# timoklein/alphazero-gym

Measured on NVIDIA B200. Metric: MCTS simulations/sec (batched trees), higher is better.
Workload: dtype f64 tree statistics + env dynamics / f32 network with exact int8-sliced tensor-core products

## Files before the change

### alphazero_gym_b200/csrc/engine.cu

```cuda
#include <cuda_runtime.h>

#include <cmath>
#include <cstdio>
#include <cstdlib>
#include <cstring>
#include <initializer_list>
#include <map>
#include <string>
#include <tuple>
#include <utility>
#include <vector>

#include "../../include/azg.h"
#include "common.cuh"
#include "env.cuh"
#include "mlp.cuh"
#include "qmlp.cuh"
#include "qmlp2.cuh"
#include "search_wg.cuh"
#include "selfplay.cuh"
#include "tree_continuous.cuh"
#include "tree_discrete.cuh"

static thread_local std::string g_err;
// ... 371 lines not shown
                volatile float tq = w[(size_t)j * H + k] * sc;
                const float tv = tq;
                int32_t q = tv != tv ? 0 : (tv >= 2147483648.0f ? INT32_MAX : (tv <= -2147483648.0f ? INT32_MIN : (int32_t)nearbyintf(tv)));
                const uint32_t t = ((uint32_t)q + 0x8080u) ^ 0x8080u;
                if (natural_rows) {
                    const size_t o = (size_t)(k / 16) * WG_B_KCHUNK + (size_t)(j / 16) * WG_B_STEP + (size_t)(j % 16) * 16 + (k % 16);
                    pl[o] = (int8_t)((t >> 16) & 0xFF);
                    pl[o + 256] = (int8_t)((t >> 8) & 0xFF);
                    pl[o + 512] = (int8_t)(t & 0xFF);
                    continue;
                }
                const size_t o = (size_t)(k / 16) * 2048 + (size_t)qmlp_perm_row(j) * 16 + (k % 16);
                pl[o] = (int8_t)((t >> 16) & 0xFF);
                pl[QMLP_PLANE + o] = (int8_t)((t >> 8) & 0xFF);
                pl[2 * QMLP_PLANE + o] = (int8_t)(t & 0xFF);
            }
        }
        d += 2 * H;
        w += (size_t)H * H + H;
    }
    const float* wv = w;
    const float* bv = w + H;
    const float* wd = w + H + 1;
    const float* bd = wd + (size_t)P * H;
    for (int k = 0; k < H; ++k) {
        d[(size_t)k * PO] = wv[k];
        for (int q = 0; q < P; ++q) d[(size_t)k * PO + 1 + q] = wd[(size_t)q * H + k];
    }
    d += (size_t)H * PO;
    d[0] = bv[0];
    for (int q = 0; q < P; ++q) d[1 + q] = bd[q];
}

extern "C" int azg_set_weights(azg_engine* e, const float* flat, int64_t n, void* stream) {
    if (!e || !flat) return fail(AZG_EINVAL, "null argument");
    if (n != e->n_weights) return fail(AZG_EINVAL, "weight count " + std::to_string(n) + " != expected " + std::to_string(e->n_weights));
    CK(cudaSetDevice(e->cfg.device));
    cudaStream_t st = (cudaStream_t)stream;
    std::vector<float> host(n);
    cudaPointerAttributes at;
    bool on_device = cudaPointerGetAttributes(&at, flat) == cudaSuccess && (at.type == cudaMemoryTypeDevice || at.type == cudaMemoryTypeManaged);
    cudaGetLastError();
    if (on_device) {
        CK(cudaMemcpyAsync(host.data(), flat, n * sizeof(float), cudaMemcpyDeviceToHost, st));
        CK(cudaStreamSynchronize(st));
    } else {
        memcpy(host.data(), flat, n * sizeof(float));
    }
    std::vector<float> packed;
    pack_weights(e, host.data(), packed);
    CK(cudaMemcpyAsync(e->wpack, packed.data(), packed.size() * sizeof(float), cudaMemcpyHostToDevice, st));
    std::vector<int8_t> qd;
    std::vector<float> qf;
    if (e->q8) {
        pack_weights_q8(e, host.data(), qd, qf);
        CK(cudaMemcpyAsync(e->qdigits, qd.data(), qd.size(), cudaMemcpyHostToDevice, st));
        std::vector<int8_t> qn;
        std::vector<float> qf2;
        pack_weights_q8(e, host.data(), qn, qf2, true);
        CK(cudaMemcpyAsync(e->qdigits_nat, qn.data(), qn.size(), cudaMemcpyHostToDevice, st));
        CK(cudaStreamSynchronize(st));
        CK(cudaMemcpyAsync(e->qfl, qf.data(), qf.size() * sizeof(float), cudaMemcpyHostToDevice, st));
    }
    CK(cudaStreamSynchronize(st));
    e->weights_set = true;
    return AZG_OK;
}

extern "C" int azg_set_tapes(azg_engine* e, const float* d_V, const float* d_prior, const float* d_action) {
    if (!e) return fail(AZG_EINVAL, "null engine");
    if (d_V) {
        if (e->cfg.variant == AZG_DISCRETE && !d_prior) return fail(AZG_EINVAL, "discrete tapes need priors");
        if (e->cfg.variant == AZG_CONTINUOUS && !d_action) return fail(AZG_EINVAL, "continuous tapes need actions");
    }
    e->tapeV = d_V;
    e->tapeP = d_V ? d_prior : nullptr;
    e->tapeA = d_V ? d_action : nullptr;
    return AZG_OK;
}

static TreeParams make_params(const azg_engine* e, int B, int64_t tree_id0) {
    TreeParams p;
    memset(&p, 0, sizeof p);
    const azg_config& c = e->cfg;
    p.B = B; p.R = e->R; p.A = c.num_actions; p.K = c.num_components; p.HS = e->HS;
    p.puct_f32 = c.puct_f32; p.v_target = c.v_target; p.use_tape = e->tapeV != nullptr;
    p.c_uct = c.c_uct; p.gamma = c.gamma; p.epsilon = c.epsilon;
    p.reward_step = e->reward_step; p.reward_terminal = e->reward_terminal;
    p.gamma_f32 = (float)c.gamma; p.action_bound = c.action_bound;
    p.seedp = e->d_seed; p.tree_id0 = tree_id0;
    p.drows = e->drows; p.dstate = e->dstate;
    p.crows = e->crows; p.et = e->et; p.ctl = e->ctl; p.BS = e->cfg.max_trees; p.chead = e->chead;
    p.pw_table = e->pw_table;
    p.rcp_tab = e->dtab; p.sqrt_tab = e->dtab + AZG_TAB + 1;
    p.n_rows = e->n_rows; p.draws = e->draws; p.leaf = e->leaf; p.path = e->path; p.dpath = e->dpath; p.ddepth = e->ddepth; p.mt = e->mt; p.tmt = e->tmt; p.rng_mt = e->mt != nullptr;
    p.ctr = e->ctr; p.X = e->X; p.root_state = e->root_state; p.root_n_init = e->root_n_init; p.err = e->err;
    p.tapeV = e->tapeV; p.tapeP = e->tapeP; p.tapeA = e->tapeA;
    p.prof = e->stats + 8;
    return p;
}

static MlpParams make_mlp_params(const azg_engine* e, int n) {
    MlpParams m;
    memset(&m, 0, sizeof m);
    const azg_config& c = e->cfg;
    m.wpack = e->wpack; m.wcount = e->wcount; m.L = c.n_hidden; m.P = e->P; m.PO_PAD = e->PO_PAD;
    m.n = n; m.X = reinterpret_cast<const float*>(e->X); m.xstride = 4; m.mode = 0;
    m.variant = c.variant; m.A = c.num_actions; m.K = c.num_components; m.R = e->R; m.HS = e->HS;
    m.ls_min = c.log_std_min; m.ls_max = c.log_std_max;
    m.leaf = e->leaf; m.drows = e->drows; m.crows = e->crows; m.chead = e->chead; m.evals = e->ctr + (size_t)3 * n;
    m.ctl = e->ctl; m.et = e->et; m.BS = c.max_trees; m.gamma_f32 = (float)c.gamma;
    m.head_dim = azg_head_dim(e);
    m.qdigits = e->qdigits; m.qdigits_nat = e->qdigits_nat; m.qfl = e->qfl; m.qfl_count = e->qfl_count;
    m.stats = e->stats;
    return m;
}

template <typename... KArgs, typename... Args>
static cudaError_t launch_ex(const azg_engine* e, void (*kernel)(KArgs...), int grid, int block, size_t smem, cudaStream_t st, Args&&... args) {
    cudaLaunchConfig_t cfg;
    memset(&cfg, 0, sizeof cfg);
    cfg.gridDim = dim3(grid);
    cfg.blockDim = dim3(block);
    cfg.dynamicSmemBytes = smem;
    cfg.stream = st;
    cfg.attrs = const_cast<cudaLaunchAttribute*>(&e->l2attr);
    cfg.numAttrs = e->l2_on ? 1 : 0;
    return cudaLaunchKernelEx(&cfg, kernel, std::forward<Args>(args)...);
}

template <int H, int S, int ACT>
static cudaError_t launch_mlp_t(const azg_engine* e, const MlpParams& m, cudaStream_t st, bool set_attr) {
    if (set_attr) return cudaFuncSetAttribute(k_mlp<H, S, ACT>, cudaFuncAttributeMaxDynamicSharedMemorySize, (int)e->mlp_smem);
    const int units = (m.n + MLP_UNIT - 1) / MLP_UNIT;
    const int grid = std::max(1, std::min((units + MLP_NGRP - 1) / MLP_NGRP, e->sm_count));
    return launch_ex(e, k_mlp<H, S, ACT>, grid, MLP_THREADS(H), e->mlp_smem, st, m);
}

template <int S, int ACT, int NL>
static cudaError_t launch_qmlp_t(const azg_engine* e, const MlpParams& m, cudaStream_t st, bool set_attr) {
    if (set_attr) {
        cudaError_t ce = cudaFuncSetAttribute(k_qmlp2<S, ACT, NL, false>, cudaFuncAttributeMaxDynamicSharedMemorySize, (int)e->qmlp_smem);
        if (ce != cudaSuccess) return ce;
        ce = cudaFuncSetAttribute(k_qmlp2<S, ACT, NL, true>, cudaFuncAttributeMaxDynamicSharedMemorySize, (int)e->qmlp_smem);
        if (ce != cudaSuccess) return ce;
        if constexpr (S == 4) {
            cudaFuncAttributes fa;
            ce = cudaFuncGetAttributes(&fa, k_qmlp2<S, ACT, NL, true, true>);
            if (ce != cudaSuccess) return ce;
            const_cast<azg_engine*>(e)->tsm_smem_max = e->smem_optin - std::min(e->smem_optin, fa.sharedSizeBytes);
            ce = cudaFuncSetAttribute(k_qmlp2<S, ACT, NL, true, true>, cudaFuncAttributeMaxDynamicSharedMemorySize, (int)e->tsm_smem_max);
            if (ce != cudaSuccess) return ce;
        }
        cudaFuncAttributes fa;
        ce = cudaFuncGetAttributes(&fa, k_search_wg<S, ACT, NL>);
        if (ce != cudaSuccess) return ce;
        if (fa.numRegs * WG_THREADS < WG_EPI_THREADS * WG_EPI_REGS + 128 * WG_MMA_REGS) return cudaErrorLaunchOutOfResources;
        return cudaFuncSetAttribute(k_search_wg<S, ACT, NL>, cudaFuncAttributeMaxDynamicSharedMemorySize, (int)e->wg_smem);
    }
    const int grid = std::max(1, std::min((m.n + 127) / 128, e->sm_count));
    TreeParams none;
    memset(&none, 0, sizeof none);
    return launch_ex(e, k_qmlp2<S, ACT, NL, false>, grid, Q2_THREADS, e->qmlp_smem, st, m, none, 0, 0, 0);
}

template <int S, int ACT, int NL>
static cudaError_t launch_fused_t(const azg_engine* e, const MlpParams& m, const TreeParams& p, int N, cudaStream_t st, int* launches) {
    int chunk = e->sm_count * Q2_MAX_TILES * 128;
    if constexpr (S == 4) {
        int cap = 0;
        while (cap < 128 && qmlp2_tsm_smem_bytes(NL, e->qfl_count, cap + 1, p.R, e->PO_PAD) <= e->tsm_smem_max) ++cap;
        const long long wave = (long long)cap * e->sm_count;
        if (cap > 0 && !p.rng_mt && !getenv("AZG_NO_TSM") && e->fused_mode != 2 && p.B > wave && p.B <= 2 * wave) chunk = (p.B + 1) / 2;
    }
    for (int lo = 0; lo < p.B; lo += chunk) {
        const int hi = std::min(p.B, lo + chunk);
        cudaError_t ce;
        const bool two_phase = e->fused_mode == 1 || (e->fused_mode == 0 && (hi - lo) < 3 * 128 * e->sm_count);
        int tsm_per = 0;
        if constexpr (S == 4) {
            const int per = (hi - lo + e->sm_count - 1) / e->sm_count;
            if (two_phase && !p.rng_mt && !getenv("AZG_NO_TSM") && per <= 128 &&
                qmlp2_tsm_smem_bytes(NL, e->qfl_count, per, p.R, e->PO_PAD) <= e->tsm_smem_max)
                tsm_per = per;
        }
        const_cast<azg_engine*>(e)->last_fused_kind = tsm_per ? 3 : (two_phase ? 1 : 2);
        if (tsm_per) {
            if constexpr (S == 4) {
                const int grid = (hi - lo + tsm_per - 1) / tsm_per;
                ce = launch_ex(e, k_qmlp2<S, ACT, NL, true, true>, grid, Q2_THREADS, qmlp2_tsm_smem_bytes(NL, e->qfl_count, tsm_per, p.R, e->PO_PAD), st, m, p, N, lo, hi);
            }
        } else if (two_phase) {
            const int grid = std::max(1, std::min((hi - lo + 127) / 128, e->sm_count));
            ce = launch_ex(e, k_qmlp2<S, ACT, NL, true>, grid, Q2_THREADS, e->qmlp_smem, st, m, p, N, lo, hi);
        } else {
            const int grid = std::max(1, std::min((hi - lo + 3) / 4, e->sm_count));
            ce = launch_ex(e, k_search_wg<S, ACT, NL>, grid, WG_THREADS, e->wg_smem, st, m, p, N, lo, hi);
        }
        ++*launches;
        if (ce != cudaSuccess) return ce;
    }
    return cudaSuccess;
}

static cudaError_t launch_fused(const azg_engine* e, const MlpParams& m, const TreeParams& p, int N, cudaStream_t st, int* launches) {
    const int S = e->cfg.state_dim, A = e->cfg.activation, NL = e->cfg.n_hidden - 1;
#define FUSED_CASE(s, a, nl) \
    if (S == s && A == a && NL == nl) return launch_fused_t<s, a, nl>(e, m, p, N, st, launches);
    FUSED_CASE(3, 0, 1) FUSED_CASE(3, 1, 1) FUSED_CASE(3, 0, 2) FUSED_CASE(3, 1, 2)
    FUSED_CASE(4, 0, 1) FUSED_CASE(4, 1, 1) FUSED_CASE(4, 0, 2) FUSED_CASE(4, 1, 2)
#undef FUSED_CASE
    return cudaErrorInvalidValue;
}

static cudaError_t launch_mlp(const azg_engine* e, const MlpParams& m, cudaStream_t st, bool set_attr) {
    const int H = e->cfg.hidden, S = e->cfg.state_dim, A = e->cfg.activation;
    if (e->q8) {
        const int NL = e->cfg.n_hidden - 1;
#define QMLP_CASE(s, a, nl) \
    if (S == s && A == a && NL == nl) return launch_qmlp_t<s, a, nl>(e, m, st, set_attr);
        QMLP_CASE(4, 0, 1) QMLP_CASE(4, 1, 1) QMLP_CASE(3, 0, 1) QMLP_CASE(3, 1, 1)
        QMLP_CASE(4, 0, 2) QMLP_CASE(4, 1, 2) QMLP_CASE(3, 0, 2) QMLP_CASE(3, 1, 2)
#undef QMLP_CASE
        return cudaErrorInvalidValue;
    }
#define MLP_CASE(h, s, a) \
    if (H == h && S == s && A == a) return launch_mlp_t<h, s, a>(e, m, st, set_attr);
    MLP_CASE(128, 4, 0) MLP_CASE(128, 4, 1) MLP_CASE(128, 3, 0) MLP_CASE(128, 3, 1)
    MLP_CASE(64, 4, 0) MLP_CASE(64, 4, 1) MLP_CASE(64, 3, 0) MLP_CASE(64, 3, 1)
    MLP_CASE(128, 4, 2) MLP_CASE(128, 4, 3) MLP_CASE(128, 4, 4) MLP_CASE(128, 4, 5)
    MLP_CASE(128, 3, 2) MLP_CASE(128, 3, 3) MLP_CASE(128, 3, 4) MLP_CASE(128, 3, 5)
    MLP_CASE(64, 4, 2) MLP_CASE(64, 4, 3) MLP_CASE(64, 4, 4) MLP_CASE(64, 4, 5)
    MLP_CASE(64, 3, 2) MLP_CASE(64, 3, 3) MLP_CASE(64, 3, 4) MLP_CASE(64, 3, 5)
#undef MLP_CASE
    return cudaErrorInvalidValue;
}

template <bool BK, bool SEL>
static cudaError_t launch_step_continuous(const azg_engine* e, const TreeParams& p, cudaStream_t st) {
    return launch_ex(e, k_step_continuous<BK, SEL>, (p.B + 127) / 128, 128, 0, st, p);
}

struct Prof {
    std::vector<cudaEvent_t> ev;
    std::vector<int> cls;
};

static int enqueue_search(azg_engine* e, int B, int N, int64_t tree_id0, cudaStream_t st, cudaError_t* cerr, Prof* prof = nullptr, bool tree_word = false) {
    TreeParams p = make_params(e, B, tree_word ? 0 : tree_id0);
    p.tree_word = tree_word ? 1 : 0;
    const MlpParams m = make_mlp_params(e, B);
    const bool tape = p.use_tape != 0;
    int launches = 0;
    cudaError_t ce = cudaSuccess;
    auto begin = [&](int cls) {
        if (!prof) return;
        cudaEvent_t a, b;
        cudaEventCreate(&a);
        cudaEventCreate(&b);
        prof->ev.push_back(a);
        prof->ev.push_back(b);
        prof->cls.push_back(cls);
        cudaEventRecord(a, st);
    };
    auto end = [&]() {
        if (prof) cudaEventRecord(prof->ev.back(), st);
    };
#define LK(cls, expr)                                   \
    do {                                                \
        begin(cls);                                     \
        expr;                                           \
        end();                                          \
        ++launches;                                     \
        if (ce == cudaSuccess) ce = cudaGetLastError(); \
    } while (0)
    const int tb = 128, tg = (B + tb - 1) / tb;
    if (e->fused && !tape && !prof) {
        ce = launch_fused(e, m, p, N, st, &launches);
        *cerr = ce;
        return launches;
    }
    if (e->cfg.variant == AZG_DISCRETE) {
        LK(2, (k_init_discrete<<<tg, tb, 0, st>>>(p)));
        if (!tape) LK(1, ce = launch_mlp(e, m, st, false));
        for (int it = 0; it < N; ++it) {
            if (it == 0) LK(0, (k_step_discrete<false, true><<<tg, tb, 0, st>>>(p)));
            else LK(0, (k_step_discrete<true, true><<<tg, tb, 0, st>>>(p)));
            if (!tape) LK(1, ce = launch_mlp(e, m, st, false));
        }
        LK(0, (k_step_discrete<true, false><<<tg, tb, 0, st>>>(p)));
    } else {
        LK(2, (k_init_continuous<<<tg, tb, 0, st>>>(p)));
        if (!tape) LK(1, ce = launch_mlp(e, m, st, false));
        LK(2, (k_root_insert_continuous<<<tg, tb, 0, st>>>(p)));
        for (int it = 0; it < N; ++it) {
            if (it == 0) LK(0, ce = (launch_step_continuous<false, true>(e, p, st)));
            else LK(0, ce = (launch_step_continuous<true, true>(e, p, st)));
            if (!tape) LK(1, ce = launch_mlp(e, m, st, false));
        }
        LK(0, ce = (launch_step_continuous<true, false>(e, p, st)));
    }
#undef LK
    *cerr = ce;
    return launches;
}

static int run_search(azg_engine* e, int B, const double* d_root_state, const int32_t* d_root_n_init, int N, int64_t tree_id0,
                      cudaStream_t st) {
    if (!e) return fail(AZG_EINVAL, "null engine");
    if (B < 1 || B > e->cfg.max_trees) return fail(AZG_EINVAL, "B out of range (max_trees = " + std::to_string(e->cfg.max_trees) + ")");
// ... 539 lines not shown
```

### alphazero_gym_b200/csrc/search_wg.cuh

```cuda
#pragma once
#include "qmlp2.cuh"

#define WG_THREADS 640
#define WG_EPI_THREADS 512
#define WG_IDESC(N) ((2u << 4) | (1u << 7) | (1u << 10) | (((uint32_t)(N) >> 3) << 17) | ((128u >> 4) << 24))
#define WG_B_KCHUNK 6144
#define WG_B_STEP 768
#define WG_WIN_COLS 48
#define WG_STASH_COL 96
#define WG_SLOT_COLS 224
#define WG_MAX_ROUNDS 4

__host__ __device__ inline size_t search_wg_smem_bytes(int NL, int qfl_count) {
    return (size_t)NL * 3 * QMLP_PLANE + 2 * 3 * QMLP_PLANE + (size_t)qfl_count * 4 + 1024 + Q2_TAB_BYTES;
}

__device__ __forceinline__ void umma_i8_wg(uint32_t tmem_d, uint32_t da_lo, uint32_t db_lo, uint32_t idesc, uint32_t accumulate) {
    asm volatile(
        "{\n\t.reg .pred p;\n\t.reg .b64 da, db;\n\tmov.b64 da, {%1, %5};\n\tmov.b64 db, {%2, %5};\n\tsetp.ne.b32 p, %4, 0;\n\t"
        "tcgen05.mma.cta_group::1.kind::i8 [%0], da, db, %3, p;\n\t}" ::"r"(tmem_d),
        "r"(da_lo), "r"(db_lo), "r"(idesc), "r"(accumulate), "r"(Q2_DESC_HI)
        : "memory");
}
__device__ __forceinline__ uint32_t wg_descb_lo(uint32_t saddr) { return ((saddr >> 4) & 0x3FFFu) | (((uint32_t)WG_B_KCHUNK >> 4) << 16); }

#ifndef WG_EPI_REGS
#define WG_EPI_REGS 104
#define WG_MMA_REGS 56
#endif

__device__ __forceinline__ void mbar_arrive_s(uint32_t bar) { asm volatile("mbarrier.arrive.shared::cta.b64 _, [%0];" ::"r"(bar) : "memory"); }
__device__ __forceinline__ bool mbar_try_wait_s(uint32_t bar, uint32_t parity, uint32_t ns) {
    uint32_t ok;
    asm volatile("{\n\t.reg .pred p;\n\tmbarrier.try_wait.parity.shared::cta.b64 p, [%1], %2, %3;\n\tselp.u32 %0, 1, 0, p;\n\t}"
                 : "=r"(ok) : "r"(bar), "r"(parity), "r"(ns) : "memory");
    return ok != 0;
}
__device__ __forceinline__ void mbar_wait_s(uint32_t bar, uint32_t parity) {
    int spins = 0;
    while (!mbar_try_wait_s(bar, parity, 20000u)) {
        if (++spins > (1 << 22)) {
            printf("mbar_wait timeout: block %d thread %d barrier smem 0x%x parity %u\n", blockIdx.x, threadIdx.x, bar, parity);
            __trap();
        }
    }
}

struct WgSlot {
    uint32_t tacc;
    int8_t* sA;
    uint32_t ready, full, accfree, slotfree;
    uint32_t fullph;
    long long cyc_full;
#ifdef AZG_EVAL_PROF
    long long cyc_k[3];
#endif
};

__device__ __forceinline__ float wg_quantise_row(const WgSlot& sl, bool wact, int r, float pm) {
    float cx = 0.0f;
    if (wact) {
        const int e = q8_exponent(pm);
        const float sx = __uint_as_float((uint32_t)(276 - e) << 23);
        cx = __uint_as_float((uint32_t)(e - 22) << 23);
#pragma unroll 2
        for (int c = 0; c < 8; ++c) {
            float v[16];
            tmem_ld16f(sl.tacc + WG_STASH_COL + 16 * c, v);
            tmem_wait_ld();
            q8_store16(v, sx, sl.sA, c, r);
        }
        asm volatile("fence.proxy.async.shared::cta;" ::: "memory");
    }
    tc_fence_before();
    mbar_arrive_s(sl.ready);
    return cx;
}

template <int S, int ACT, int NL>
__device__ __forceinline__ void wg_evaluate(const MlpParams& p, WgSlot& sl, const float* fl, bool wact, bool valid, int gr, int r, float* out) {
    const float* W0 = fl;
    const float* b0 = fl + S * 128;
    const float2* cwb = reinterpret_cast<const float2*>(fl + S * 128 + 128);
    const float* Wh = fl + S * 128 + 128 + NL * 2 * 128;
    const float* bh = Wh + 128 * p.PO_PAD;
    float pm = 0.0f;
    if (wact) {
        float x[S];
#pragma unroll
        for (int s = 0; s < S; ++s) x[s] = 0.0f;
        if (valid) {
            const float4 v = *reinterpret_cast<const float4*>(p.X + (size_t)gr * 4);
            x[0] = v.x; x[1] = v.y; x[2] = v.z;
            if (S > 3) x[S - 1] = v.w;
        }
#pragma unroll 1
        for (int c = 0; c < 8; ++c) {
            float a[16];
#pragma unroll
            for (int i = 0; i < 16; i += 2) {
                const int j = c * 16 + i;
                float2 acc = *reinterpret_cast<const float2*>(b0 + j);
#pragma unroll
                for (int s = 0; s < S; ++s) acc = __ffma2_rn(make_float2(x[s], x[s]), *reinterpret_cast<const float2*>(W0 + s * 128 + j), acc);
                const float2 e = mlp_act2<ACT>(acc);
                a[i] = e.x; a[i + 1] = e.y;
                pm = fmaxf(pm, fmaxf(fabsf(e.x), fabsf(e.y)));
            }
            tmem_st16f(sl.tacc + WG_STASH_COL + 16 * c, a);
        }
        tmem_wait_st();
    }
    float cx = wg_quantise_row(sl, wact, r, pm);
#pragma unroll 1
    for (int l = 0; l < NL; ++l) {
        pm = 0.0f;
#pragma unroll 1
        for (int k = 0; k < 8; ++k) {
            const int w = k & 1;
            const long long f0 = clock64();
            mbar_wait_s(sl.full + 8u * w, (sl.fullph >> w) & 1u);
            sl.fullph ^= 1u << w;
            tc_fence_after();
            sl.cyc_full += clock64() - f0;
#ifdef AZG_EVAL_PROF
            sl.cyc_k[k < 2 ? k : 2] += clock64() - f0;
#endif
            if (wact) {
                const uint32_t ta = sl.tacc + w * WG_WIN_COLS;
                int32_t pa[16], pb[16], pc[16];
                tmem_ld16(ta, pa);
                tmem_ld16(ta + 16, pb);
                tmem_ld16(ta + 32, pc);
                tmem_wait_ld();
                tc_fence_before();
                if (k < 6) mbar_arrive_s(sl.accfree + 8u * w);
                const float2* cb = cwb + l * 128 + 16 * k;
                float v[16];
#pragma unroll
                for (int i = 0; i < 16; i += 2) {
                    const float4 sb = *reinterpret_cast<const float4*>(cb + i);
                    float u0 = __int2float_rn(pa[i] * 256 + pb[i]);
                    float u1 = __int2float_rn(pa[i + 1] * 256 + pb[i + 1]);
                    u0 = __fmaf_rn(u0, 256.0f, q8_i2f_23(pc[i]));
                    u1 = __fmaf_rn(u1, 256.0f, q8_i2f_23(pc[i + 1]));
                    const float2 y = make_float2(__fmaf_rn(u0, __fmul_rn(cx, sb.x), sb.y), __fmaf_rn(u1, __fmul_rn(cx, sb.z), sb.w));
                    const float2 ev = mlp_act2<ACT>(y);
                    v[i] = ev.x; v[i + 1] = ev.y;
                    pm = fmaxf(pm, fmaxf(fabsf(ev.x), fabsf(ev.y)));
                }
                tmem_st16f(sl.tacc + WG_STASH_COL + 16 * k, v);
            } else {
                tc_fence_before();
                if (k < 6) mbar_arrive_s(sl.accfree + 8u * w);
            }
        }
        if (wact) tmem_wait_st();
        if (l + 1 < NL) cx = wg_quantise_row(sl, wact, r, pm);
    }
    if (wact) {
#pragma unroll 1
        for (int c4 = 0; c4 < p.PO_PAD / 4; ++c4) {
            float2 lo[4], hi[4];
#pragma unroll
            for (int q = 0; q < 4; ++q) {
                lo[q] = make_float2(0.0f, 0.0f);
                hi[q] = make_float2(0.0f, 0.0f);
#pragma unroll
                for (int hc = 0; hc < 2; ++hc) {
                    float a[16];
                    tmem_ld16f(sl.tacc + WG_STASH_COL + 32 * q + 16 * hc, a);
                    tmem_wait_ld();
                    const float* wp = Wh + (32 * q + 16 * hc) * p.PO_PAD + c4 * 4;
#pragma unroll
                    for (int i = 0; i < 16; ++i) {
                        const float4 w4 = *reinterpret_cast<const float4*>(wp + i * p.PO_PAD);
                        const float2 av = make_float2(a[i], a[i]);
                        lo[q] = __ffma2_rn(av, make_float2(w4.x, w4.y), lo[q]);
                        hi[q] = __ffma2_rn(av, make_float2(w4.z, w4.w), hi[q]);
                    }
                }
            }
            const float s0 = __fadd_rn(__fadd_rn(__fadd_rn(lo[0].x, lo[1].x), __fadd_rn(lo[2].x, lo[3].x)), bh[c4 * 4 + 0]);
            const float s1 = __fadd_rn(__fadd_rn(__fadd_rn(lo[0].y, lo[1].y), __fadd_rn(lo[2].y, lo[3].y)), bh[c4 * 4 + 1]);
            const float s2 = __fadd_rn(__fadd_rn(__fadd_rn(hi[0].x, hi[1].x), __fadd_rn(hi[2].x, hi[3].x)), bh[c4 * 4 + 2]);
            const float s3 = __fadd_rn(__fadd_rn(__fadd_rn(hi[0].y, hi[1].y), __fadd_rn(hi[2].y, hi[3].y)), bh[c4 * 4 + 3]);
#pragma unroll
            for (int g4 = 0; g4 < Q2_MAX_PO / 4; ++g4)
                if (g4 == c4) { out[4 * g4] = s0; out[4 * g4 + 1] = s1; out[4 * g4 + 2] = s2; out[4 * g4 + 3] = s3; }
        }
    }
    tc_fence_before();
}

template <int S, int ACT, int NL>
__global__ void __launch_bounds__(WG_THREADS, 1)
k_search_wg(const MlpParams p, const TreeParams tp, const int n_sims, const int chunk_begin, const int chunk_end) {
    extern __shared__ __align__(1024) uint8_t wsm_raw[];
    __shared__ __align__(8) uint64_t wbar, ready[2], full[2][2], accfree[2][2], slotfree[2][2];
    __shared__ uint32_t tmem_base_s;
    uint8_t* qsm = wsm_raw + ((1024u - (smem_u32(wsm_raw) & 1023u)) & 1023u);
    int8_t* sB = reinterpret_cast<int8_t*>(qsm);
    int8_t* sA = sB + (size_t)NL * 3 * QMLP_PLANE;
    float* fl = reinterpret_cast<float*>(sA + 2 * 3 * QMLP_PLANE);
    double* s_rcp = reinterpret_cast<double*>(fl + p.qfl_count);
    double* s_sq = s_rcp + FUSED_TAB + 1;
    int32_t* s_pw = reinterpret_cast<int32_t*>(s_sq + FUSED_TAB + 1);

    const int tid = threadIdx.x, warp = tid >> 5, lane = tid & 31;
    const int per = (chunk_end - chunk_begin + gridDim.x - 1) / gridDim.x;
    const int row_begin = chunk_begin + blockIdx.x * per;
    const int row_end = min(row_begin + per, chunk_end);
    if (row_begin >= row_end) return;
    const int nrows = row_end - row_begin;
    const int rounds = (nrows + 511) / 512;
    const int ntiles_max = 4 * rounds;
    int th = (nrows + ntiles_max - 1) / ntiles_max;
    if (th > 32) th = (th + 31) & ~31;
    const int ntiles = (nrows + th - 1) / th;
    const int n_evals = n_sims + 1;

    if (tid == 0) {
        mbar_init(&wbar, 1);
        for (int s = 0; s < 2; ++s) {
            mbar_init(&ready[s], 128);
            mbar_init(&slotfree[s][0], 128);
            mbar_init(&slotfree[s][1], 128);
            for (int w = 0; w < 2; ++w) {
                mbar_init(&full[s][w], 1);
                mbar_init(&accfree[s][w], 128);
            }
        }
    }
    if (warp == 0) {
        asm volatile("tcgen05.alloc.cta_group::1.sync.aligned.shared::cta.b32 [%0], %1;" ::"r"(smem_u32(&tmem_base_s)), "n"(512) : "memory");
        asm volatile("tcgen05.relinquish_alloc_permit.cta_group::1.sync.aligned;" ::: "memory");
    }
    tc_fence_before();
    __syncthreads();
    tc_fence_after();
    const uint32_t tb = tmem_base_s;
#ifdef AZG_WG_DEBUG
    if (tid == 0 && blockIdx.x == 0)
        printf("wg: wbar 0x%x ready 0x%x full 0x%x accfree 0x%x slotfree 0x%x tmem 0x%x nrows %d th %d ntiles %d rounds %d\n", smem_u32(&wbar), smem_u32(ready),
               smem_u32(&full[0][0]), smem_u32(&accfree[0][0]), smem_u32(&slotfree[0][0]), tb, nrows, th, ntiles, rounds);
#endif
    if (tid == 0) {
        const uint32_t bytesB = (uint32_t)NL * 3 * QMLP_PLANE, bytesF = (uint32_t)p.qfl_count * 4u;
        mbar_expect_tx(&wbar, bytesB + bytesF);
        for (uint32_t o = 0; o < bytesB; o += 32768u) bulk_g2s(sB + o, p.qdigits_nat + o, min(32768u, bytesB - o), &wbar);
        bulk_g2s(fl, p.qfl, bytesF, &wbar);
    }
    for (int i = tid; i <= FUSED_TAB; i += blockDim.x) {
        s_rcp[i] = tp.rcp_tab[i];
        s_sq[i] = tp.sqrt_tab[i];
        s_pw[i] = (tp.pw_table && i < p.R) ? tp.pw_table[i] : 0;
    }
    __syncthreads();
    mbar_wait(&wbar, 0);

    if (warp >= 16) {
        asm volatile("setmaxnreg.dec.sync.aligned.u32 %0;" ::"n"(WG_MMA_REGS));
        if (warp < 18) {
            const int slot = warp - 16;
            uint32_t rph = 0, aph = 0;
            const uint32_t aH = q2_desc_lo(smem_u32(sA) + (uint32_t)slot * 3 * QMLP_PLANE), aM = aH + 1024, aL = aH + 2048;
#pragma unroll 1
            for (int s = 0; s < n_evals; ++s)
#pragma unroll 1
            for (int rd = 0; rd < rounds; ++rd)
#pragma unroll 1
            for (int half = 0; half < 2; ++half) {
                if (4 * rd + slot + 2 * half >= ntiles) continue;
#pragma unroll 1
                for (int l = 0; l < NL; ++l) {
#pragma unroll 1
                    for (int k = 0; k < 8; ++k) {
                        const int w = k & 1;
                        if (k == 0) { mbar_wait(&ready[slot], rph); rph ^= 1u; }
                        else if (k >= 2) { mbar_wait(&accfree[slot][w], (aph >> w) & 1u); aph ^= 1u << w; }
                        tc_fence_after();
                        const uint32_t bq = wg_descb_lo(smem_u32(sB) + (uint32_t)l * 3 * QMLP_PLANE + (uint32_t)k * WG_B_STEP);
                        const uint32_t acc = tb + slot * WG_SLOT_COLS + w * WG_WIN_COLS;
                        if (elect_one()) {
#pragma unroll
                        for (int kk = 0; kk < 4; ++kk) {
                            umma_i8_wg(acc, aH + kk * 256, bq + kk * 768, WG_IDESC(48), kk > 0);
                            umma_i8_wg(acc + 16, aM + kk * 256, bq + kk * 768, WG_IDESC(32), 1);
                            umma_i8_wg(acc + 32, aL + kk * 256, bq + kk * 768, WG_IDESC(16), 1);
                        }
                        umma_commit(&full[slot][w]);
                        }
                        __syncwarp();
                    }
                }
            }
        }
    } else {
        asm volatile("setmaxnreg.inc.sync.aligned.u32 %0;" ::"n"(WG_EPI_REGS));
        const int g = warp >> 2, slot = g & 1, half = g >> 1;
        const int r = (warp & 3) * 32 + lane;
        WgSlot sl;
        sl.tacc = tb + ((uint32_t)((warp & 3) * 32) << 16) + slot * WG_SLOT_COLS;
        sl.sA = sA + (size_t)slot * 3 * QMLP_PLANE;
        sl.ready = smem_u32(&ready[slot]); sl.full = smem_u32(full[slot]); sl.accfree = smem_u32(accfree[slot]); sl.slotfree = smem_u32(slotfree[slot]);
        sl.fullph = 0;
        sl.cyc_full = 0;
#ifdef AZG_EVAL_PROF
        sl.cyc_k[0] = sl.cyc_k[1] = sl.cyc_k[2] = 0;
#endif
        bool first_use = true;
        uint32_t useph = 0;
        const Tabs tabs = {s_pw, s_rcp, s_sq, FUSED_TAB};
        long long cyc_tree = 0, cyc_slot = 0;
        const long long cyc_begin = clock64();
        uint32_t nev = 0;
        int ev_row = 0;
        for (int rd = 0; rd < rounds; ++rd) {
            const int tile = 4 * rd + g, row0 = row_begin + tile * th;
            if (tile < ntiles && row0 + r < min(row0 + th, row_end)) {
                if (S == 4) d_init(tp, row0 + r);
                else c_init(tp, row0 + r);
            }
        }
#pragma unroll 1
        for (int s = 0; s < n_evals; ++s) {
#pragma unroll 1
        for (int rd = 0; rd < rounds; ++rd) {
            const int tile = 4 * rd + g;
            const bool tvalid = tile < ntiles;
            const int row0 = row_begin + tile * th;
            const int nv = tvalid ? max(0, min(th, row_end - row0)) : 0;
            const int gr = row0 + r;
            const bool valid = r < nv, wact = (warp & 3) * 32 < nv;
            const long long c0 = clock64();
            if (half == 1 || !first_use) {
                mbar_wait_s(sl.slotfree + 8u * (half ^ 1), useph);
                useph ^= 1u;
            }
            first_use = false;
            tc_fence_after();
            const long long c1 = clock64();
            float out[Q2_MAX_PO];
#pragma unroll
            for (int i = 0; i < Q2_MAX_PO; ++i) out[i] = 0.0f;
            if (tvalid) wg_evaluate<S, ACT, NL>(p, sl, fl, wact, valid, gr, r, out);
            mbar_arrive_s(sl.slotfree + 8u * half);
            const long long c2 = clock64();
            if (valid) {
                int leafw;
                double lr = 0.0;
                if (p.variant == 1) {
                    const uint4 k0 = p.ctl[gr], k1 = p.ctl[(size_t)p.BS + gr];
                    leafw = (int)k0.z;
                    lr = __hiloint2double((int)k1.w, (int)k1.z);
                } else {
                    leafw = p.leaf[gr];
                }
                if (leafw & LEAF_EVAL) {
                    mlp_finish_row(p, gr, leafw, lr, out[0], out + 1);
                    ++nev;
                    ev_row = gr;
                }
                if (S == 4) {
                    d_step(tp, tabs, gr, s > 0, s + 1 < n_evals);
                } else {
                    if (s == 0) c_root_insert(tp, gr);
                    c_step(tp, tabs, gr, s > 0, s + 1 < n_evals);
                }
            }
            cyc_slot += c1 - c0;
            cyc_tree += clock64() - c2;
        }
        }
        if (nev) p.evals[ev_row] += nev;
        if ((warp & 3) == 0 && lane == 0 && p.stats) {
            atomicAdd(p.stats + 0, (unsigned long long)(clock64() - cyc_begin));
            atomicAdd(p.stats + 1, (unsigned long long)cyc_tree);
            atomicAdd(p.stats + 2, (unsigned long long)cyc_slot);
            atomicAdd(p.stats + 3, (unsigned long long)sl.cyc_full);
#ifdef AZG_EVAL_PROF
            for (int k = 0; k < 3; ++k) atomicAdd(p.stats + 8 + k, (unsigned long long)sl.cyc_k[k]);
#endif
            atomicAdd(p.stats + 4, 1ull);
        }
    }
    tc_fence_before();
    __syncthreads();
    if (warp == 0) asm volatile("tcgen05.dealloc.cta_group::1.sync.aligned.b32 %0, %1;" ::"r"(tb), "n"(512) : "memory");
}
```

Baseline: 1.146 billion.

## Remove dedicated MMA warps; last-arriving epilogue warp issues tcgen05 MMAs

Drops the two producer warps and the setmaxnreg split (640→512 threads). MMA issue now happens in whichever epilogue warp is the fourth to arrive, detected through a shared-memory atomic counter per slot, which replaces the ready/accfree mbarriers. Separately, when PO_PAD ≤ 8 the last hidden layer is fused with the head projection in registers, so that layer's activations are no longer stashed to TMEM. The aims are to cut warp handoff latency and register pressure, at the cost of MMA issue work sitting on the epilogue critical path and the counter logic needing to stay correct.

```diff
diff --git a/alphazero_gym_b200/csrc/engine.cu b/alphazero_gym_b200/csrc/engine.cu
--- a/alphazero_gym_b200/csrc/engine.cu
+++ b/alphazero_gym_b200/csrc/engine.cu
@@ -547,10 +547,6 @@
             ce = cudaFuncSetAttribute(k_qmlp2<S, ACT, NL, true, true>, cudaFuncAttributeMaxDynamicSharedMemorySize, (int)e->tsm_smem_max);
             if (ce != cudaSuccess) return ce;
         }
-        cudaFuncAttributes fa;
-        ce = cudaFuncGetAttributes(&fa, k_search_wg<S, ACT, NL>);
-        if (ce != cudaSuccess) return ce;
-        if (fa.numRegs * WG_THREADS < WG_EPI_THREADS * WG_EPI_REGS + 128 * WG_MMA_REGS) return cudaErrorLaunchOutOfResources;
         return cudaFuncSetAttribute(k_search_wg<S, ACT, NL>, cudaFuncAttributeMaxDynamicSharedMemorySize, (int)e->wg_smem);
     }
     const int grid = std::max(1, std::min((m.n + 127) / 128, e->sm_count));
diff --git a/alphazero_gym_b200/csrc/search_wg.cuh b/alphazero_gym_b200/csrc/search_wg.cuh
--- a/alphazero_gym_b200/csrc/search_wg.cuh
+++ b/alphazero_gym_b200/csrc/search_wg.cuh
@@ -1,8 +1,7 @@
 #pragma once
 #include "qmlp2.cuh"
 
-#define WG_THREADS 640
-#define WG_EPI_THREADS 512
+#define WG_THREADS 512
 #define WG_IDESC(N) ((2u << 4) | (1u << 7) | (1u << 10) | (((uint32_t)(N) >> 3) << 17) | ((128u >> 4) << 24))
 #define WG_B_KCHUNK 6144
 #define WG_B_STEP 768
@@ -24,11 +23,6 @@
 }
 __device__ __forceinline__ uint32_t wg_descb_lo(uint32_t saddr) { return ((saddr >> 4) & 0x3FFFu) | (((uint32_t)WG_B_KCHUNK >> 4) << 16); }
 
-#ifndef WG_EPI_REGS
-#define WG_EPI_REGS 104
-#define WG_MMA_REGS 56
-#endif
-
 __device__ __forceinline__ void mbar_arrive_s(uint32_t bar) { asm volatile("mbarrier.arrive.shared::cta.b64 _, [%0];" ::"r"(bar) : "memory"); }
 __device__ __forceinline__ bool mbar_try_wait_s(uint32_t bar, uint32_t parity, uint32_t ns) {
     uint32_t ok;
@@ -49,7 +43,9 @@
 struct WgSlot {
     uint32_t tacc;
     int8_t* sA;
-    uint32_t ready, full, accfree, slotfree;
+    uint32_t sB;
+    uint32_t ctr;
+    uint32_t full, slotfree;
     uint32_t fullph;
     long long cyc_full;
 #ifdef AZG_EVAL_PROF
@@ -57,7 +53,32 @@
 #endif
 };
 
-__device__ __forceinline__ float wg_quantise_row(const WgSlot& sl, bool wact, int r, float pm) {
+__device__ __forceinline__ void wg_arrive(const WgSlot& sl, int c, int l, int k0, int k1) {
+    __syncwarp();
+    uint32_t old = 0;
+    if ((threadIdx.x & 31) == 0)
+        asm volatile("atom.acq_rel.cta.shared::cta.add.u32 %0, [%1], 1;" : "=r"(old) : "r"(sl.ctr + 4u * c) : "memory");
+    if ((__shfl_sync(0xffffffffu, old, 0) & 3u) != 3u) return;
+    tc_fence_after();
+    const uint32_t aH = q2_desc_lo(smem_u32(sl.sA)), aM = aH + 1024, aL = aH + 2048;
+#pragma unroll 1
+    for (int k = k0; k < k1; ++k) {
+        const uint32_t bq = wg_descb_lo(sl.sB + (uint32_t)l * 3 * QMLP_PLANE + (uint32_t)k * WG_B_STEP);
+        const uint32_t acc = (sl.tacc & 0xFFFFu) + (k & 1) * WG_WIN_COLS;
+        if (elect_one()) {
+#pragma unroll
+            for (int kk = 0; kk < 4; ++kk) {
+                umma_i8_wg(acc, aH + kk * 256, bq + kk * 768, WG_IDESC(48), kk > 0);
+                umma_i8_wg(acc + 16, aM + kk * 256, bq + kk * 768, WG_IDESC(32), 1);
+                umma_i8_wg(acc + 32, aL + kk * 256, bq + kk * 768, WG_IDESC(16), 1);
+            }
+            asm volatile("tcgen05.commit.cta_group::1.mbarrier::arrive::one.shared::cluster.b64 [%0];" ::"r"(sl.full + 8u * (k & 1)) : "memory");
+        }
+        __syncwarp();
+    }
+}
+
+__device__ __forceinline__ float wg_quantise_row(const WgSlot& sl, bool wact, int r, float pm, int l) {
     float cx = 0.0f;
     if (wact) {
         const int e = q8_exponent(pm);
@@ -73,8 +94,88 @@
         asm volatile("fence.proxy.async.shared::cta;" ::: "memory");
     }
     tc_fence_before();
-    mbar_arrive_s(sl.ready);
+    wg_arrive(sl, 0, l, 0, 2);
     return cx;
+}
+
+template <int ACT, bool FOLD>
+__device__ __forceinline__ void wg_layer(const MlpParams& p, WgSlot& sl, const float2* cwb, const float* Wh, const float* bh, bool wact, int l,
+                                         float cx, float& pm, float* out) {
+    float2 h[4], qa[4], qb[4];
+    pm = 0.0f;
+#pragma unroll 1
+    for (int k = 0; k < 8; ++k) {
+        const int w = k & 1;
+        const long long f0 = clock64();
+        mbar_wait_s(sl.full + 8u * w, (sl.fullph >> w) & 1u);
+        sl.fullph ^= 1u << w;
+        tc_fence_after();
+        sl.cyc_full += clock64() - f0;
+#ifdef AZG_EVAL_PROF
+        sl.cyc_k[k < 2 ? k : 2] += clock64() - f0;
+#endif
+        float u[16];
+        if (wact) {
+            const uint32_t ta = sl.tacc + w * WG_WIN_COLS;
+            int32_t pa[16], pb[16], pc[16];
+            tmem_ld16(ta, pa);
+            tmem_ld16(ta + 16, pb);
+            tmem_ld16(ta + 32, pc);
+            tmem_wait_ld();
+#pragma unroll
+            for (int i = 0; i < 16; ++i) u[i] = __fmaf_rn(__int2float_rn(pa[i] * 256 + pb[i]), 256.0f, q8_i2f_23(pc[i]));
+        }
+        tc_fence_before();
+        if (k < 6) wg_arrive(sl, 1 + w, l, k + 2, k + 3);
+        if (!wact) continue;
+        const float2* cb = cwb + l * 128 + 16 * k;
+        float v[16];
+#pragma unroll
+        for (int i = 0; i < 16; i += 2) {
+            const float4 sb = *reinterpret_cast<const float4*>(cb + i);
+            const float2 y = make_float2(__fmaf_rn(u[i], __fmul_rn(cx, sb.x), sb.y), __fmaf_rn(u[i + 1], __fmul_rn(cx, sb.z), sb.w));
+            const float2 ev = mlp_act2<ACT>(y);
+            v[i] = ev.x; v[i + 1] = ev.y;
+            if (!FOLD) pm = fmaxf(pm, fmaxf(fabsf(ev.x), fabsf(ev.y)));
+        }
+        if (!FOLD) {
+            tmem_st16f(sl.tacc + WG_STASH_COL + 16 * k, v);
+            continue;
+        }
+        if ((k & 1) == 0) h[0] = h[1] = h[2] = h[3] = make_float2(0.0f, 0.0f);
+        const float* wp = Wh + 16 * k * p.PO_PAD;
+#pragma unroll
+        for (int i = 0; i < 16; ++i) {
+            const float4 w4 = *reinterpret_cast<const float4*>(wp + i * p.PO_PAD);
+            const float2 av = make_float2(v[i], v[i]);
+            h[0] = __ffma2_rn(av, make_float2(w4.x, w4.y), h[0]);
+            h[1] = __ffma2_rn(av, make_float2(w4.z, w4.w), h[1]);
+        }
+        if (p.PO_PAD > 4) {
+#pragma unroll
+            for (int i = 0; i < 16; ++i) {
+                const float4 w4 = *reinterpret_cast<const float4*>(wp + i * p.PO_PAD + 4);
+                const float2 av = make_float2(v[i], v[i]);
+                h[2] = __ffma2_rn(av, make_float2(w4.x, w4.y), h[2]);
+                h[3] = __ffma2_rn(av, make_float2(w4.z, w4.w), h[3]);
+            }
+        }
+#pragma unroll
+        for (int j = 0; j < 4; ++j) {
+            if (k == 1) qa[j] = h[j];
+            else if (k == 3) qa[j] = make_float2(__fadd_rn(qa[j].x, h[j].x), __fadd_rn(qa[j].y, h[j].y));
+            else if (k == 5) qb[j] = h[j];
+        }
+    }
+    if (!FOLD && wact) tmem_wait_st();
+    if (FOLD && wact) {
+#pragma unroll
+        for (int j = 0; j < 4; ++j) {
+            if (j >= 2 && p.PO_PAD <= 4) break;
+            out[2 * j] = __fadd_rn(__fadd_rn(qa[j].x, __fadd_rn(qb[j].x, h[j].x)), bh[2 * j]);
+            out[2 * j + 1] = __fadd_rn(__fadd_rn(qa[j].y, __fadd_rn(qb[j].y, h[j].y)), bh[2 * j + 1]);
+        }
+    }
 }
 
 template <int S, int ACT, int NL>
@@ -111,54 +212,15 @@
         }
         tmem_wait_st();
     }
-    float cx = wg_quantise_row(sl, wact, r, pm);
-#pragma unroll 1
-    for (int l = 0; l < NL; ++l) {
-        pm = 0.0f;
-#pragma unroll 1
-        for (int k = 0; k < 8; ++k) {
-            const int w = k & 1;
-            const long long f0 = clock64();
-            mbar_wait_s(sl.full + 8u * w, (sl.fullph >> w) & 1u);
-            sl.fullph ^= 1u << w;
-            tc_fence_after();
-            sl.cyc_full += clock64() - f0;
-#ifdef AZG_EVAL_PROF
-            sl.cyc_k[k < 2 ? k : 2] += clock64() - f0;
-#endif
-            if (wact) {
-                const uint32_t ta = sl.tacc + w * WG_WIN_COLS;
-                int32_t pa[16], pb[16], pc[16];
-                tmem_ld16(ta, pa);
-                tmem_ld16(ta + 16, pb);
-                tmem_ld16(ta + 32, pc);
-                tmem_wait_ld();
-                tc_fence_before();
-                if (k < 6) mbar_arrive_s(sl.accfree + 8u * w);
-                const float2* cb = cwb + l * 128 + 16 * k;
-                float v[16];
-#pragma unroll
-                for (int i = 0; i < 16; i += 2) {
-                    const float4 sb = *reinterpret_cast<const float4*>(cb + i);
-                    float u0 = __int2float_rn(pa[i] * 256 + pb[i]);
-                    float u1 = __int2float_rn(pa[i + 1] * 256 + pb[i + 1]);
-                    u0 = __fmaf_rn(u0, 256.0f, q8_i2f_23(pc[i]));
-                    u1 = __fmaf_rn(u1, 256.0f, q8_i2f_23(pc[i + 1]));
-                    const float2 y = make_float2(__fmaf_rn(u0, __fmul_rn(cx, sb.x), sb.y), __fmaf_rn(u1, __fmul_rn(cx, sb.z), sb.w));
-                    const float2 ev = mlp_act2<ACT>(y);
-                    v[i] = ev.x; v[i + 1] = ev.y;
-                    pm = fmaxf(pm, fmaxf(fabsf(ev.x), fabsf(ev.y)));
-                }
-                tmem_st16f(sl.tacc + WG_STASH_COL + 16 * k, v);
-            } else {
-                tc_fence_before();
-                if (k < 6) mbar_arrive_s(sl.accfree + 8u * w);
-            }
-        }
-        if (wact) tmem_wait_st();
-        if (l + 1 < NL) cx = wg_quantise_row(sl, wact, r, pm);
-    }
-    if (wact) {
+    float cx = wg_quantise_row(sl, wact, r, pm, 0);
+    const bool fold = p.PO_PAD <= 8;
+#pragma unroll 1
+    for (int l = 0; l < NL - (fold ? 1 : 0); ++l) {
+        wg_layer<ACT, false>(p, sl, cwb, Wh, bh, wact, l, cx, pm, out);
+        if (l + 1 < NL) cx = wg_quantise_row(sl, wact, r, pm, l + 1);
+    }
+    if (fold) wg_layer<ACT, true>(p, sl, cwb, Wh, bh, wact, NL - 1, cx, pm, out);
+    if (wact && !fold) {
 #pragma unroll 1
         for (int c4 = 0; c4 < p.PO_PAD / 4; ++c4) {
             float2 lo[4], hi[4];
@@ -197,7 +259,8 @@
 __global__ void __launch_bounds__(WG_THREADS, 1)
 k_search_wg(const MlpParams p, const TreeParams tp, const int n_sims, const int chunk_begin, const int chunk_end) {
     extern __shared__ __align__(1024) uint8_t wsm_raw[];
-    __shared__ __align__(8) uint64_t wbar, ready[2], full[2][2], accfree[2][2], slotfree[2][2];
+    __shared__ __align__(8) uint64_t wbar, full[2][2], slotfree[2][2];
+    __shared__ uint32_t ctr[2][3];
     __shared__ uint32_t tmem_base_s;
     uint8_t* qsm = wsm_raw + ((1024u - (smem_u32(wsm_raw) & 1023u)) & 1023u);
     int8_t* sB = reinterpret_cast<int8_t*>(qsm);
@@ -223,13 +286,10 @@
     if (tid == 0) {
         mbar_init(&wbar, 1);
         for (int s = 0; s < 2; ++s) {
-            mbar_init(&ready[s], 128);
             mbar_init(&slotfree[s][0], 128);
             mbar_init(&slotfree[s][1], 128);
-            for (int w = 0; w < 2; ++w) {
-                mbar_init(&full[s][w], 1);
-                mbar_init(&accfree[s][w], 128);
-            }
+            for (int w = 0; w < 2; ++w) mbar_init(&full[s][w], 1);
+            for (int c = 0; c < 3; ++c) ctr[s][c] = 0;
         }
     }
     if (warp == 0) {
@@ -242,8 +302,8 @@
     const uint32_t tb = tmem_base_s;
 #ifdef AZG_WG_DEBUG
     if (tid == 0 && blockIdx.x == 0)
-        printf("wg: wbar 0x%x ready 0x%x full 0x%x accfree 0x%x slotfree 0x%x tmem 0x%x nrows %d th %d ntiles %d rounds %d\n", smem_u32(&wbar), smem_u32(ready),
-               smem_u32(&full[0][0]), smem_u32(&accfree[0][0]), smem_u32(&slotfree[0][0]), tb, nrows, th, ntiles, rounds);
+        printf("wg: wbar 0x%x ctr 0x%x full 0x%x slotfree 0x%x tmem 0x%x nrows %d th %d ntiles %d rounds %d\n", smem_u32(&wbar), smem_u32(ctr),
+               smem_u32(&full[0][0]), smem_u32(&slotfree[0][0]), tb, nrows, th, ntiles, rounds);
 #endif
     if (tid == 0) {
         const uint32_t bytesB = (uint32_t)NL * 3 * QMLP_PLANE, bytesF = (uint32_t)p.qfl_count * 4u;
@@ -259,131 +319,92 @@
     __syncthreads();
     mbar_wait(&wbar, 0);
 
-    if (warp >= 16) {
-        asm volatile("setmaxnreg.dec.sync.aligned.u32 %0;" ::"n"(WG_MMA_REGS));
-        if (warp < 18) {
-            const int slot = warp - 16;
-            uint32_t rph = 0, aph = 0;
-            const uint32_t aH = q2_desc_lo(smem_u32(sA) + (uint32_t)slot * 3 * QMLP_PLANE), aM = aH + 1024, aL = aH + 2048;
-#pragma unroll 1
-            for (int s = 0; s < n_evals; ++s)
-#pragma unroll 1
-            for (int rd = 0; rd < rounds; ++rd)
-#pragma unroll 1
-            for (int half = 0; half < 2; ++half) {
-                if (4 * rd + slot + 2 * half >= ntiles) continue;
-#pragma unroll 1
-                for (int l = 0; l < NL; ++l) {
-#pragma unroll 1
-                    for (int k = 0; k < 8; ++k) {
-                        const int w = k & 1;
-                        if (k == 0) { mbar_wait(&ready[slot], rph); rph ^= 1u; }
-                        else if (k >= 2) { mbar_wait(&accfree[slot][w], (aph >> w) & 1u); aph ^= 1u << w; }
-                        tc_fence_after();
-                        const uint32_t bq = wg_descb_lo(smem_u32(sB) + (uint32_t)l * 3 * QMLP_PLANE + (uint32_t)k * WG_B_STEP);
-                        const uint32_t acc = tb + slot * WG_SLOT_COLS + w * WG_WIN_COLS;
-                        if (elect_one()) {
-#pragma unroll
-                        for (int kk = 0; kk < 4; ++kk) {
-                            umma_i8_wg(acc, aH + kk * 256, bq + kk * 768, WG_IDESC(48), kk > 0);
-                            umma_i8_wg(acc + 16, aM + kk * 256, bq + kk * 768, WG_IDESC(32), 1);
-                            umma_i8_wg(acc + 32, aL + kk * 256, bq + kk * 768, WG_IDESC(16), 1);
-                        }
-                        umma_commit(&full[slot][w]);
-                        }
-                        __syncwarp();
-                    }
-                }
-            }
-        }
-    } else {
-        asm volatile("setmaxnreg.inc.sync.aligned.u32 %0;" ::"n"(WG_EPI_REGS));
-        const int g = warp >> 2, slot = g & 1, half = g >> 1;
-        const int r = (warp & 3) * 32 + lane;
-        WgSlot sl;
-        sl.tacc = tb + ((uint32_t)((warp & 3) * 32) << 16) + slot * WG_SLOT_COLS;
-        sl.sA = sA + (size_t)slot * 3 * QMLP_PLANE;
-        sl.ready = smem_u32(&ready[slot]); sl.full = smem_u32(full[slot]); sl.accfree = smem_u32(accfree[slot]); sl.slotfree = smem_u32(slotfree[slot]);
-        sl.fullph = 0;
-        sl.cyc_full = 0;
+    const int g = warp >> 2, slot = g & 1, half = g >> 1;
+    const int r = (warp & 3) * 32 + lane;
+    WgSlot sl;
+    sl.tacc = tb + ((uint32_t)((warp & 3) * 32) << 16) + slot * WG_SLOT_COLS;
+    sl.sA = sA + (size_t)slot * 3 * QMLP_PLANE;
+    sl.sB = smem_u32(sB);
+    sl.ctr = smem_u32(ctr[slot]); sl.full = smem_u32(full[slot]); sl.slotfree = smem_u32(slotfree[slot]);
+    sl.fullph = 0;
+    sl.cyc_full = 0;
 #ifdef AZG_EVAL_PROF
-        sl.cyc_k[0] = sl.cyc_k[1] = sl.cyc_k[2] = 0;
+    sl.cyc_k[0] = sl.cyc_k[1] = sl.cyc_k[2] = 0;
 #endif
-        bool first_use = true;
-        uint32_t useph = 0;
-        const Tabs tabs = {s_pw, s_rcp, s_sq, FUSED_TAB};
-        long long cyc_tree = 0, cyc_slot = 0;
-        const long long cyc_begin = clock64();
-        uint32_t nev = 0;
-        int ev_row = 0;
-        for (int rd = 0; rd < rounds; ++rd) {
-            const int tile = 4 * rd + g, row0 = row_begin + tile * th;
-            if (tile < ntiles && row0 + r < min(row0 + th, row_end)) {
-                if (S == 4) d_init(tp, row0 + r);
-                else c_init(tp, row0 + r);
-            }
-        }
-#pragma unroll 1
-        for (int s = 0; s < n_evals; ++s) {
-#pragma unroll 1
-        for (int rd = 0; rd < rounds; ++rd) {
-            const int tile = 4 * rd + g;
-            const bool tvalid = tile < ntiles;
-            const int row0 = row_begin + tile * th;
-            const int nv = tvalid ? max(0, min(th, row_end - row0)) : 0;
-            const int gr = row0 + r;
-            const bool valid = r < nv, wact = (warp & 3) * 32 < nv;
-            const long long c0 = clock64();
-            if (half == 1 || !first_use) {
-                mbar_wait_s(sl.slotfree + 8u * (half ^ 1), useph);
-                useph ^= 1u;
-            }
-            first_use = false;
-            tc_fence_after();
-            const long long c1 = clock64();
-            float out[Q2_MAX_PO];
-#pragma unroll
-            for (int i = 0; i < Q2_MAX_PO; ++i) out[i] = 0.0f;
-            if (tvalid) wg_evaluate<S, ACT, NL>(p, sl, fl, wact, valid, gr, r, out);
-            mbar_arrive_s(sl.slotfree + 8u * half);
-            const long long c2 = clock64();
-            if (valid) {
-                int leafw;
-                double lr = 0.0;
-                if (p.variant == 1) {
-                    const uint4 k0 = p.ctl[gr], k1 = p.ctl[(size_t)p.BS + gr];
-                    leafw = (int)k0.z;
-                    lr = __hiloint2double((int)k1.w, (int)k1.z);
-                } else {
-                    leafw = p.leaf[gr];
-                }
-                if (leafw & LEAF_EVAL) {
-                    mlp_finish_row(p, gr, leafw, lr, out[0], out + 1);
-                    ++nev;
-                    ev_row = gr;
-                }
-                if (S == 4) {
-                    d_step(tp, tabs, gr, s > 0, s + 1 < n_evals);
-                } else {
-                    if (s == 0) c_root_insert(tp, gr);
-                    c_step(tp, tabs, gr, s > 0, s + 1 < n_evals);
-                }
-            }
-            cyc_slot += c1 - c0;
-            cyc_tree += clock64() - c2;
-        }
-        }
-        if (nev) p.evals[ev_row] += nev;
-        if ((warp & 3) == 0 && lane == 0 && p.stats) {
-            atomicAdd(p.stats + 0, (unsigned long long)(clock64() - cyc_begin));
-            atomicAdd(p.stats + 1, (unsigned long long)cyc_tree);
-            atomicAdd(p.stats + 2, (unsigned long long)cyc_slot);
-            atomicAdd(p.stats + 3, (unsigned long long)sl.cyc_full);
+    bool first_use = true;
+    uint32_t useph = 0;
+    const Tabs tabs = {s_pw, s_rcp, s_sq, FUSED_TAB};
+    long long cyc_tree = 0, cyc_slot = 0;
+    const long long cyc_begin = clock64();
+    uint32_t nev = 0;
+    int ev_row = 0;
+    for (int rd = 0; rd < rounds; ++rd) {
+        const int tile = 4 * rd + g, row0 = row_begin + tile * th;
+        if (tile < ntiles && row0 + r < min(row0 + th, row_end)) {
+            if (S == 4) d_init(tp, row0 + r);
+            else c_init(tp, row0 + r);
+        }
+    }
+#pragma unroll 1
+    for (int s = 0; s < n_evals; ++s) {
+#pragma unroll 1
+    for (int rd = 0; rd < rounds; ++rd) {
+        const int tile = 4 * rd + g;
+        const bool tvalid = tile < ntiles;
+        const int row0 = row_begin + tile * th;
+        const int nv = tvalid ? max(0, min(th, row_end - row0)) : 0;
+        const int gr = row0 + r;
+        const bool valid = r < nv, wact = (warp & 3) * 32 < nv;
+        const long long c0 = clock64();
+        if (half == 1 || !first_use) {
+            mbar_wait_s(sl.slotfree + 8u * (half ^ 1), useph);
+            useph ^= 1u;
+        }
+        first_use = false;
+        tc_fence_after();
+        const long long c1 = clock64();
+        float out[Q2_MAX_PO];
+#pragma unroll
+        for (int i = 0; i < Q2_MAX_PO; ++i) out[i] = 0.0f;
+        if (tvalid) wg_evaluate<S, ACT, NL>(p, sl, fl, wact, valid, gr, r, out);
+        mbar_arrive_s(sl.slotfree + 8u * half);
+        const long long c2 = clock64();
+        if (valid) {
+            int leafw;
+            double lr = 0.0;
+            if (p.variant == 1) {
+                const uint4 k0 = p.ctl[gr], k1 = p.ctl[(size_t)p.BS + gr];
+                leafw = (int)k0.z;
+                lr = __hiloint2double((int)k1.w, (int)k1.z);
+            } else {
+                leafw = p.leaf[gr];
+            }
+            if (leafw & LEAF_EVAL) {
+                mlp_finish_row(p, gr, leafw, lr, out[0], out + 1);
+                ++nev;
+                ev_row = gr;
+            }
+            if (S == 4) {
+                d_step(tp, tabs, gr, s > 0, s + 1 < n_evals);
+            } else {
+                if (s == 0) c_root_insert(tp, gr);
+                c_step(tp, tabs, gr, s > 0, s + 1 < n_evals);
+            }
+        }
+        cyc_slot += c1 - c0;
+        cyc_tree += clock64() - c2;
+    }
+    }
+    if (nev) p.evals[ev_row] += nev;
+    if ((warp & 3) == 0 && lane == 0 && p.stats) {
+        atomicAdd(p.stats + 0, (unsigned long long)(clock64() - cyc_begin));
+        atomicAdd(p.stats + 1, (unsigned long long)cyc_tree);
+        atomicAdd(p.stats + 2, (unsigned long long)cyc_slot);
+        atomicAdd(p.stats + 3, (unsigned long long)sl.cyc_full);
 #ifdef AZG_EVAL_PROF
-            for (int k = 0; k < 3; ++k) atomicAdd(p.stats + 8 + k, (unsigned long long)sl.cyc_k[k]);
+        for (int k = 0; k < 3; ++k) atomicAdd(p.stats + 8 + k, (unsigned long long)sl.cyc_k[k]);
 #endif
-            atomicAdd(p.stats + 4, 1ull);
-        }
+        atomicAdd(p.stats + 4, 1ull);
     }
     tc_fence_before();
     __syncthreads();
```

After: 804.0 million (median of 6 runs). 29.9% lower.
